# szpajder/dumphfdl

Measured on AMD Instinct MI355X. Metric: wideband I/Q Msamples/s (cf32 ingest -> decoded HFDL PDUs) at fixed channel count, higher is better.
Workload: dtype f32

## Files before the change

dumphfdl_amd/csrc/demod.h:

```cpp
#pragma once
#include <hip/hip_runtime.h>
#include <cstdint>
#include <cstddef>
#include <memory>
#include <vector>
#include "../../include/hfdl_gpu.h"
#include "hip_handles.h"
#include "kernels.h"

namespace hfdl {

struct ChanState;
struct ChanScalars;
struct FrameRec;

struct DemodImage;

struct Demod {
	int nch = 0, outs = 0, cap = 0;
	int batch = 1;
	uint32_t taken = 0, dropped = 0;
	uint64_t launches = 0, decodes = 0;
	bool separate_decode = false;
	int bounce_cap = 0;
	int pdu_cap = 0;
	bool taps_on = true;
	bool taps_enabled = true;
	size_t lds_bytes = 0;
	Stream st_collect;
	std::unique_ptr<DemodImage> img;
	DevBuf d_tables;
	DevArray<ChanState> d_states;
	DevArray<float2> d_data;
	DevArray<FrameRec> d_frames;
	DevArray<int> d_counts;
// ... 35 lines not shown
```

dumphfdl_amd/csrc/demod_core.h:

```cpp
#pragma once
#include <hip/hip_runtime.h>
#include "demod_logic.h"
#include "demod_lds.h"

namespace hfdl {

constexpr int DM_WAVES = 4, DM_THREADS = 64 * DM_WAVES;
constexpr int WAVE_AGC = 0, WAVE_TIMING = 1, WAVE_CARRIER = 2, WAVE_RESAMPLER = 3;

__device__ __forceinline__ float dpp_row_shr1(float old, float src)
{
	return __int_as_float(__builtin_amdgcn_update_dpp(__float_as_int(old), __float_as_int(src), 0x111, 0xf, 0xf, false));
}
__device__ __forceinline__ float dpp_row_shl1(float old, float src)
{
	return __int_as_float(__builtin_amdgcn_update_dpp(__float_as_int(old), __float_as_int(src), 0x101, 0xf, 0xf, false));
}
__device__ __forceinline__ float dpp_row_shl2(float old, float src)
{
	return __int_as_float(__builtin_amdgcn_update_dpp(__float_as_int(old), __float_as_int(src), 0x102, 0xf, 0xf, false));
}
__device__ __forceinline__ float dpp_row_ror1(float src)
{
	return __int_as_float(__builtin_amdgcn_update_dpp(0, __float_as_int(src), 0x121, 0xf, 0xf, false));
// ... 139 lines not shown
		io.mf[p] = v;
		if (p >= DM_RING - SS_HIST) io.mf[p - DM_RING] = v;
		if (TAPS) { io.tap_mf[k] = v; io.tap_level[k] = io.lvl[p]; }
	}
}


struct DemodInput {
	const cf *chan;
	size_t blk_stride;
	const int *ends;
	cf *ring;
	int n_in;
};

__device__ __forceinline__ cf input_sample(const DemodInput &in, int g)
{
	int b = 0, start = 0;
#pragma unroll
	for (int u = 0; u < DM_MAX_BLOCKS - 1; u++) {
		const int e = in.ends[u];
		if (g >= e) { b = u + 1; start = e; }
	}
	return in.chan[(size_t)b * in.blk_stride + (size_t)(g - start)];
}

template <bool TAPS>
__device__ __forceinline__ void resample_outputs(uint32_t rs_phase, const DemodConst &T, const BlockIo &io, const cf *ring, int k0, int k1, int lane)
{
	const int k = k0 + lane;
	if (k < k1) {
		const uint64_t t = (uint64_t)rs_phase + (uint64_t)k * T.rs_step;
		const int i = (int)(t >> 24);
		const float *h = T.rs_h + ((t & 0xFFFFFFu) >> 16) * D_RS_TAPS;
		float ar = 0, ai = 0;
		for (int j = 0; j < D_RS_TAPS; j++) {
			const cf x = ring[(i - j) & DM_IN_MASK];
// ... 501 lines not shown
	auto resampler_store = [&]() {
		cf nh;
		if (lane < D_RS_TAPS - 1) nh = in.ring[(n_in - 1 - lane) & DM_IN_MASK];
		__builtin_amdgcn_wave_barrier();
		if (lane < D_RS_TAPS - 1) a.rs_hist[lane] = nh;
		if (lane == 0) {
			S.rs_phase = (uint32_t)((uint64_t)rs_phase + (uint64_t)n_out * T.rs_step - total);
			if (TAPS) io.tap_counts[0] = n_out;
		}
	};

	if (tid < D_RS_TAPS - 1) in.ring[(-1 - tid) & DM_IN_MASK] = a.rs_hist[tid];
	if (wave == WAVE_TIMING && lane < D_MF - 1) io.agc[(-1 - lane) & DM_AGC_MASK] = a.mf_hist[lane];
	const int rs0 = n_out < DM_CHUNK ? n_out : DM_CHUNK;
	int in_loaded = need(rs0 + 2 * DM_CHUNK);
	for (int g = tid; g < in_loaded; g += DM_THREADS) in.ring[g & DM_IN_MASK] = input_sample(in, g);
	if (TAPS && tid == 0) io.tap_counts[1] = 0;
	__syncthreads();
	if (wave == WAVE_RESAMPLER) resample_outputs<TAPS>(rs_phase, T, io, in.ring, 0, rs0, lane);
	__syncthreads();
	if (n_out < 1) {
		if (wave == WAVE_RESAMPLER) resampler_store();
		return 0;
	}

	unsigned long long tP0 = __builtin_amdgcn_s_memtime();
	unsigned long long busy = 0;
	int nsym = 0;
	StepClock clk;
	StateProbe states;
	PipeProgress pp;
	pp.rs_ready = rs0;
	if (wave == WAVE_RESAMPLER) {
		for (int step = 0; pp.s3_done < n_out; step++) {
			PipeMail &mail = step_mail(sh.mbox, step);
			clk.begin<WAVE_RESAMPLER>();
			int to = pp.rs_ready;
			if (to < n_out) {
				to = resampler_advance(pp, n_out);
				const int hi = need(resampler_fetch_ahead(to, n_out));
				cf nx[2];
#pragma unroll
				for (int u = 0; u < 2; u++) {
					const int g = in_loaded + 64 * u + lane;
					nx[u] = g < hi ? input_sample(in, g) : cf{0.f, 0.f};
				}
				resample_outputs<TAPS>(rs_phase, T, io, in.ring, pp.rs_ready, to, lane);
#pragma unroll
				for (int u = 0; u < 2; u++) {
					const int g = in_loaded + 64 * u + lane;
					if (g < hi) in.ring[g & DM_IN_MASK] = nx[u];
				}
				for (int g = in_loaded + 128 + lane; g < hi; g += 64) in.ring[g & DM_IN_MASK] = input_sample(in, g);
				if (hi > in_loaded) in_loaded = hi;
			}
			if (lane == 0) mail.rs_ready = to;
			clk.end<WAVE_RESAMPLER>(busy, mail, lane);
			__syncthreads();
			pp.read(&mail);
		}
		resampler_store();
	} else if (wave == WAVE_AGC) {
		float agc_g = S.agc_g, agc_y2 = S.agc_y2;
		for (int step = 0; pp.s3_done < n_out; step++) {
			PipeMail &mail = step_mail(sh.mbox, step);
			clk.begin<WAVE_AGC>();
			int to = agc_advance(pp);
			if (to > pp.mf_ready) agc_mf_chunk<TAPS>(agc_g, agc_y2, T, io, pp.mf_ready, to, lane); else to = pp.mf_ready;
// ... 78 lines not shown
```

dumphfdl_amd/csrc/demod_host.cpp:

```cpp
#include <algorithm>
#include <cmath>
#include <cstdlib>
#include <cstring>
#include <vector>
#include "demod.h"
#include "demod_launch.h"
#include "demod_lds.h"
#include "demod_tables.h"

namespace hfdl {

struct DemodImage { DemodTables h; DevTables t; };

Demod::Demod() = default;
Demod::~Demod() = default;

static DevTables resolve_tables(const void *d_img, const DemodTables &h)
{
	const unsigned char *base = (const unsigned char *)d_img;
	auto at = [&](const void *field) { return base + ((const unsigned char *)field - (const unsigned char *)&h); };
	DevTables t;
	t.c.rs_h = (const float *)at(h.rs_h);
	t.c.rs_step = h.rs_step;
	t.c.mf = (const float *)at(h.mf);
// ... 1 lines not shown
	t.c.ss_dmf = (const float *)at(h.ss_dmf);
	t.c.lf_b0 = h.lf_b0; t.c.lf_a1 = h.lf_a1; t.c.ss_rate_adj = h.ss_rate_adj;
	t.c.eq_h0 = (const float *)at(h.eq_h0);
	t.c.a_hi = h.a_hi; t.c.a_lo = h.a_lo;
	t.c.m1_hi = (const uint64_t *)at(h.m1_hi);
	t.c.m1_lo = (const uint64_t *)at(h.m1_lo);
	t.scrambler = (const uint8_t *)at(h.scrambler);
	t.c.corr_tab = (const float *)at(h.corr_tab);
	t.c.psk_pts = (const float *)at(h.psk_pts);
	t.c.a1_lo = h.a1_lo; t.c.a1_hi = h.a1_hi; t.c.a2_lo = h.a2_lo; t.c.a2_hi = h.a2_hi; t.c.pos_min = h.pos_min;
	return t;
}

size_t Demod::workgroup_lds() { return demod_workgroup_lds(0); }

int Demod::fit_batch(int outs, float resamp_rate, int want)
{
	int batch = want < 1 ? 1 : (want > DM_MAX_BLOCKS ? DM_MAX_BLOCKS : want);
	for (;; batch--) {
		const int cap = (int)((double)outs * (double)batch * (double)resamp_rate + 8);
		if (batch > 1 && demod_workgroup_lds(cap) > 160 * 1024) continue;
		if (batch == 1 || (2 * cap <= 65535 && (double)cap / 5400.0 < 1.0)) break;
	}
	return batch;
}

int Demod::init(int nch_, int outs_, float resamp_rate, const int32_t *freqs, hipStream_t st, int batch_want)
{
	nch = nch_; outs = outs_;
	if (resamp_rate <= 0.5f || resamp_rate > 1.0f) return fail(HFDL_GPU_ERANGE, "resampling rate %g outside (0.5, 1]", (double)resamp_rate);
	batch = fit_batch(outs, resamp_rate, batch_want);
	cap = (int)((double)outs * (double)batch * (double)resamp_rate + 8);
	img = std::make_unique<DemodImage>();
	build_demod_tables(img->h, resamp_rate);
	CREATE_TRY(d_tables.alloc(sizeof(DemodTables)));
	CREATE_TRY(hipMemcpyAsync(d_tables.p, &img->h, sizeof(DemodTables), hipMemcpyHostToDevice, st));
	img->t = resolve_tables(d_tables.p, img->h);

	std::vector<ChanState> init((size_t)nch);
	for (auto &s : init) chan_state_init(s, img->h.eq_h0);
	CREATE_TRY(d_states.alloc((size_t)nch));
	CREATE_TRY(hipMemcpy(d_states, init.data(), sizeof(ChanState) * (size_t)nch, hipMemcpyHostToDevice));
	CREATE_TRY(d_data.alloc((size_t)nch * 2 * MAX_DATA_SYMBOLS));
	CREATE_TRY(hipMemsetAsync(d_data, 0, sizeof(float2) * (size_t)nch * 2 * MAX_DATA_SYMBOLS, st));
	CREATE_TRY(d_frames.alloc(2 * (size_t)nch));
	CREATE_TRY(d_counts.alloc(8));
	CREATE_TRY(hipMemsetAsync(d_counts, 0, sizeof(int) * 8, st));
	CREATE_TRY(h_snap.alloc(8));
	std::memset(h_snap.p, 0, sizeof(int) * 8);
	taken = 0; dropped = 0;
	pdu_cap = std::max(4096, 64 * nch);
	if (const char *e = getenv("HFDL_GPU_PDU_RING")) {
		const long v = strtol(e, nullptr, 10);
		if (v >= 1 && v <= (1 << 20)) pdu_cap = (int)v;
	}
	CREATE_TRY(d_pdus.alloc((size_t)pdu_cap));
	CREATE_TRY(st_collect.create());
	bounce_cap = pdu_cap < 512 ? pdu_cap : 512;
	CREATE_TRY(h_pdu_bounce.alloc((size_t)bounce_cap));
	CREATE_TRY(h_stats_bounce.alloc((size_t)nch));
// ... 7 lines not shown
		CREATE_TRY(d_tap_counts.alloc(2 * (size_t)nch));
		CREATE_TRY(hipMemsetAsync(d_tap_counts, 0, sizeof(int) * 2 * (size_t)nch, st));
	}
	lds_bytes = demod_workgroup_lds(cap);
	if (lds_bytes > 160 * 1024) return fail(HFDL_GPU_ERANGE, "a demodulator launch of %d samples needs %zu bytes of LDS", cap, lds_bytes);
	return prepare_demod_kernels(lds_bytes);
}

int Demod::enqueue_demod(const float2 *chan_out, const int *out_count, int nblk, hipStream_t st, hipEvent_t done, bool frames_free, hipEvent_t start)
{
	if (!img || nblk < 1 || nblk > batch || nblk > DM_MAX_BLOCKS)
		return fail(HFDL_GPU_EINVAL, "demodulator launch of %d blocks: 1 .. %d", nblk, batch);
	DemodBuffers B;
	const uint64_t i = launches++;
	if (separate_decode && !frames_free && ev_dec[i & 1]) HIP_TRY(hipStreamWaitEvent(st, ev_dec[i & 1], 0));
	B.states = d_states; B.data = (cf *)d_data.p; B.frames = d_frames + (size_t)(i & 1) * nch; B.counts = d_counts;
	B.frame_count = d_counts + 4 + (int)(i & 3); B.frame_cap = nch;
	const bool tw = taps_on && taps_enabled;
	B.tap_rs = tw ? (cf *)d_tap_rs.p : nullptr; B.tap_mf = (cf *)d_tap_mf.p; B.tap_sym = (cf *)d_tap_sym.p; B.tap_lvl = d_tap_lvl; B.tap_counts = d_tap_counts;
	B.cap = cap;
	launch_demod(tw, img->t, B, (const cf *)chan_out, out_count, outs, nblk, nch, lds_bytes, st, start, done);
	HIP_TRY(hipGetLastError());
	return 0;
}

int Demod::enqueue_decode(int buf, hipStream_t st, hipEvent_t start, hipEvent_t stop)
{
	if (!img) return fail(HFDL_GPU_EINVAL, "burst decoder launch before init");
	const uint64_t i = decodes++;
	if (i + 1 != launches) return fail(HFDL_GPU_EINVAL, "burst decoder launch %llu without its demodulator launch", (unsigned long long)i);
	launch_burst_decode(d_frames + (size_t)(i & 1) * nch, d_counts, d_counts + 4 + (int)(i & 3), d_counts + 4 + (int)((i + 2) & 3), nch,
			(const cf *)d_data.p, img->t.scrambler, d_freqs, d_pdus, pdu_cap, st, start, stop);
	HIP_TRY(hipMemcpyAsync(h_snap.p + 4 * (buf & 1), d_counts, sizeof(int) * 4, hipMemcpyDeviceToHost, st));
	if (separate_decode) {
		if (!ev_dec[i & 1]) HIP_TRY(ev_dec[i & 1].create(EV_NO_TIMING));
		HIP_TRY(hipEventRecord(ev_dec[i & 1], st));
	}
	HIP_TRY(hipGetLastError());
	return 0;
}

int Demod::prepare_retune(hipStream_t st_b)
{
	if (d_state_image.p) return 0;
	DevArray<ChanState> d;
	PinnedBuf<ChanState> h;
	Event ev;
// ... 122 lines not shown
```

dumphfdl_amd/csrc/demod_kernels.hip:

```cpp
#include <hip/hip_ext.h>
#include <utility>
#include "demod_core.h"
#ifdef HFDL_DM_STRICT
#include HFDL_DM_SERIAL_LOOP
#endif
#include "demod_tables.h"
#include "hip_handles.h"
#include "demod_launch.h"
#ifdef HFDL_LAB
#include "../../include/hfdl_gpu_lab.h"
#endif

namespace hfdl {

static_assert(sizeof(cf) == sizeof(float2), "cf must alias float2");

template <int NT, typename T>
__device__ __forceinline__ void stage_copy(T *__restrict__ dst, const T *__restrict__ src, int n, int tid)
{
	int i = tid;
	for (; i + 7 * NT < n; i += 8 * NT) {
		T v[8];
#pragma unroll
		for (int u = 0; u < 8; u++) v[u] = src[i + u * NT];
// ... 55 lines not shown
	if (tid < 8) { l_m1[tid] = T.c.m1_hi[tid]; l_m1[8 + tid] = T.c.m1_lo[tid]; }
	if (tid < 128) l_corr[tid] = T.c.corr_tab[tid];
	if (tid < (int)(2 * sizeof(PipeMail) / sizeof(int))) ((int *)(lds + L.mbox))[tid] = 0;
	__syncthreads();
	if (tid < DM_MAX_BLOCKS) {
		int sum = 0;
		for (int u = 0; u <= tid; u++) sum += l_blk[u];
		l_blk[DM_MAX_BLOCKS + tid] = sum;
	}
	__syncthreads();

	DemodConst K = T.c;
	K.rs_h = l_rs_h; K.ss_mf = nullptr; K.ss_dmf = nullptr; K.mf = l_mf; K.eq_h0 = l_eq; K.m1_hi = l_m1; K.m1_lo = l_m1 + 8; K.corr_tab = l_corr;
	BlockIo io;
	io.rs = (cf *)(lds + L.rs); io.agc = (cf *)(lds + L.agc); io.mf = (cf *)(lds + L.mfo); io.lvl = (float *)(lds + L.lvl); io.cap = B.cap;
	io.data = B.data + (size_t)c * 2 * MAX_DATA_SYMBOLS;
	io.frames = B.frames; io.frame_count = B.frame_count; io.frame_cap = B.frame_cap;
	io.channel = c;
	DemodInput in;
	in.chan = chan_out + (size_t)c * outs_stride; in.blk_stride = (size_t)nch * outs_stride;
	in.ends = l_blk + DM_MAX_BLOCKS; in.ring = (cf *)(lds + L.in); in.n_in = l_blk[2 * DM_MAX_BLOCKS - 1];
	if (TAPS) {
		io.tap_resampled = B.tap_rs + (size_t)c * B.cap; io.tap_mf = B.tap_mf + (size_t)c * B.cap;
		io.tap_symbols = B.tap_sym + (size_t)c * B.cap; io.tap_level = B.tap_lvl + (size_t)c * B.cap;
		io.tap_counts = B.tap_counts + 2 * c;
	} else {
		io.tap_resampled = nullptr; io.tap_mf = nullptr; io.tap_symbols = nullptr; io.tap_level = nullptr; io.tap_counts = nullptr;
	}
	DemodShared sh;
	sh.outq = (cf *)(lds + L.outq); sh.outq_cap = 2 * B.cap;
	sh.cum = (uint16_t *)(lds + L.cum);
// ... 167 lines not shown
	size_t table, vin, decw, consts, total;
	__host__ __device__ constexpr explicit BurstLds(bool viterbi)
		: table(0), vin(K5_TABLE_BYTES), decw(2 * (size_t)K5_TABLE_BYTES), consts(decw + (viterbi ? viterbi_lds_bytes(K5_MAX_BITS) : 0)), total(consts + DEC_CONST_BYTES) {}
};

struct BurstFrame {
	FrameRec fr;
	ModeParams mp;
	int nsym, ncoded, cols;
	const cf *sym;
	float mask_flip;
	uint8_t *l_scr;
	float *l_psk;
};

__device__ __forceinline__ BurstFrame burst_frame(const FrameRec *__restrict__ frames, int f, const cf *__restrict__ data_all, const uint8_t *__restrict__ scrambler,
		unsigned char *consts, int lane)
{
	BurstFrame b;
	b.l_scr = consts;
	b.l_psk = (float *)(consts + DEC_PSK_OFFSET);
	b.fr = frames[f];
	b.mp = mode_params(b.fr.mode);
	b.nsym = b.mp.segments * 30; b.ncoded = b.nsym * b.mp.arity; b.cols = b.ncoded / 40;
	b.sym = data_all + ((size_t)b.fr.channel * 2 + b.fr.slot) * MAX_DATA_SYMBOLS;
	b.mask_flip = b.fr.bitmask_lsb ? -1.0f : 1.0f;
	b.l_scr[lane] = lane < 120 ? scrambler[lane] : 0;
	if (lane + 64 < 120) b.l_scr[lane + 64] = scrambler[lane + 64];
	if (lane < 32) b.l_psk[lane] = ((const float *)(scrambler + DEC_PSK_OFFSET))[lane];
	__syncthreads();
	return b;
}

__device__ __forceinline__ int burst_soft_wave(const int mode, const int nsym, const int ncoded, const int cols, const cf *sym, const float mask_flip,
		const uint8_t *l_scr, const float *l_psk, uint8_t *table, uint8_t *vin)
{
	const int lane = threadIdx.x;
	const ModeParams mp = mode_params(mode);
	for (int base = 0; base < nsym; base += 256) {
		cf xs[4];
// ... 20 lines not shown
	__syncthreads();
	const int vin_len = mp.code_rate == 4 ? ncoded / 2 : ncoded;
	for (int j = lane; j < vin_len; j += 64) {
		if (mp.code_rate == 4) {
			const int p0 = 2 * j, p1 = 2 * j + 1;
			const uint8_t a = table[((9 * p0) % 40) * cols + p0 / 40], b = table[((9 * p1) % 40) * cols + p1 / 40];
			vin[j] = (uint8_t)((a & b) + ((a ^ b) >> 1));
		} else {
			vin[j] = table[((9 * j) % 40) * cols + j / 40];
		}
	}
	return vin_len;
}

__global__ __launch_bounds__(64) void burst_decode_kernel(const FrameRec *__restrict__ frames, int *counts, const int *nframes_ptr, int *stale_count, int frame_cap,
		const cf *__restrict__ data_all, const uint8_t *__restrict__ scrambler, const int32_t *__restrict__ freqs,
		hfdl_gpu_pdu *__restrict__ pdus, int pdu_cap)
{
	extern __shared__ __attribute__((aligned(16))) unsigned char lds[];
	__builtin_amdgcn_s_setprio(2);
	const int f = blockIdx.x, lane = threadIdx.x;
	int nframes = *nframes_ptr;
	if (f == 0 && lane == 0 && stale_count) *stale_count = 0;
	if (nframes > frame_cap) nframes = frame_cap;
	if (f >= nframes) return;
	constexpr BurstLds L(true);
	uint8_t *table = lds + L.table, *vin = lds + L.vin;
	uint64_t *decw = (uint64_t *)(lds + L.decw);
	const BurstFrame b = burst_frame(frames, f, data_all, scrambler, lds + L.consts, lane);
	const FrameRec &fr = b.fr;
	const ModeParams &mp = b.mp;
	const int vin_len = burst_soft_wave(fr.mode, b.nsym, b.ncoded, b.cols, b.sym, b.mask_flip, b.l_scr, b.l_psk, table, vin);
	int slot = -1;
	if (lane == 0) {
		unsigned *produced = (unsigned *)&counts[1];
		const unsigned taken = *(volatile unsigned *)&counts[3];
		unsigned t = *(volatile unsigned *)produced;
		for (;;) {
			if (t - taken >= (unsigned)pdu_cap) { atomicAdd(&counts[2], 1); break; }
			const unsigned seen = atomicCAS(produced, t, t + 1u);
			if (seen == t) { slot = (int)(t % (unsigned)pdu_cap); break; }
			t = seen;
		}
	}
// ... 29 lines not shown
		if (out->fcs_status == 0 && kind != 0) lc = lpdu_walk(l_oct, (uint32_t)noct, kind, hdr_len);
		out->lpdus_processed = lc.processed; out->lpdus_good = lc.good; out->lpdus_bad_fcs = lc.bad_fcs;
		out->lpdus_too_short = lc.too_short; out->lpdus_truncated = lc.truncated;
		out->lpdu_pad[0] = out->lpdu_pad[1] = out->lpdu_pad[2] = 0;
	}
}

#ifdef HFDL_LAB
__global__ __launch_bounds__(64) void burst_soft_kernel(const FrameRec *__restrict__ frames, const cf *__restrict__ data_all, const uint8_t *__restrict__ scrambler,
		uint8_t *__restrict__ vin_out, int32_t *__restrict__ vin_lens)
{
	extern __shared__ __attribute__((aligned(16))) unsigned char lds[];
	const int f = blockIdx.x, lane = threadIdx.x;
	constexpr BurstLds L(false);
	uint8_t *table = lds + L.table, *vin = lds + L.vin;
	const BurstFrame b = burst_frame(frames, f, data_all, scrambler, lds + L.consts, lane);
	const int vin_len = burst_soft_wave(b.fr.mode, b.nsym, b.ncoded, b.cols, b.sym, b.mask_flip, b.l_scr, b.l_psk, table, vin);
	__syncthreads();
	uint8_t *dst = vin_out + (size_t)f * HFDL_GPU_LAB_VIN_MAX;
	for (int j = lane; j < vin_len && j < HFDL_GPU_LAB_VIN_MAX; j += 64) dst[j] = vin[j];
	if (lane == 0) vin_lens[f] = vin_len;
}
#endif

__global__ __launch_bounds__(64) void viterbi_batch_kernel(const uint8_t *__restrict__ soft, int nbits, uint8_t *__restrict__ out)
{
	extern __shared__ __attribute__((aligned(16))) unsigned char lds[];
	const int f = blockIdx.x;
	viterbi27_wave(soft + (size_t)f * 2 * nbits, nbits, (uint64_t *)lds, out + (size_t)f * ((nbits + 7) / 8), false);
}

// ... 88 lines not shown
int prepare_demod_kernels(size_t demod_lds)
{
	int rc;
	if ((rc = set_big_lds((const void *)demod_kernel<true>, demod_lds))) return rc;
	if ((rc = set_big_lds((const void *)demod_kernel<false>, demod_lds))) return rc;
	return prepare_burst_decode();
}

void launch_demod(bool taps, const DevTables &T, const DemodBuffers &B, const cf *chan_out, const int *n_in, int outs_stride, int nblk, int nch,
		size_t lds, hipStream_t st, hipEvent_t start, hipEvent_t stop)
{
	if (taps) hipExtLaunchKernelGGL(demod_kernel<true>, dim3((unsigned)nch), dim3(DM_THREADS), (unsigned)lds, st, start, stop, 0, T, B, chan_out, n_in, outs_stride, nblk, nch);
	else hipExtLaunchKernelGGL(demod_kernel<false>, dim3((unsigned)nch), dim3(DM_THREADS), (unsigned)lds, st, start, stop, 0, T, B, chan_out, n_in, outs_stride, nblk, nch);
}

void launch_burst_decode(const FrameRec *frames, int *counts, const int *nframes, int *stale_count, int frame_cap, const cf *data,
		const uint8_t *scrambler, const int32_t *freqs, hfdl_gpu_pdu *pdus, int pdu_cap, hipStream_t st, hipEvent_t start, hipEvent_t stop)
{
	hipExtLaunchKernelGGL(burst_decode_kernel, dim3((unsigned)frame_cap), dim3(64), (unsigned)burst_decode_lds(), st, start, stop, 0, frames, counts,
			nframes, stale_count, frame_cap, data, scrambler, freqs, pdus, pdu_cap);
}

void launch_retune_demod(ChanState *states, const ChanState *image, int c, hipStream_t st, hipEvent_t done)
{
	hipExtLaunchKernelGGL(retune_demod_kernel, dim3(1), dim3(256), 0, st, nullptr, done, 0, states, image, c);
}

void launch_retune_freq(int32_t *freqs, int c, int32_t freq, hipStream_t st)
{
	hipLaunchKernelGGL(retune_freq_kernel, dim3(1), dim3(64), 0, st, freqs, c, freq);
}


int prepare_viterbi_batch(int nbits)
{
// ... 59 lines not shown
```

dumphfdl_amd/csrc/demod_launch.h:

```cpp
#pragma once
#include <hip/hip_runtime.h>
#include "../../include/hfdl_gpu.h"
#include "demod_logic.h"
#include "kernels.h"

namespace hfdl {

struct DevTables {
	DemodConst c;
	const uint8_t *scrambler;
};

struct DemodBuffers {
	ChanState *states;
	cf *data;
	FrameRec *frames;
	int *counts;
	int *frame_count;
	int frame_cap;
	cf *tap_rs, *tap_mf, *tap_sym;
	float *tap_lvl;
	int *tap_counts;
	int cap;
};

size_t demod_workgroup_lds(int cap);
size_t burst_decode_lds();
int prepare_demod_kernels(size_t demod_lds);
int prepare_burst_decode();
void launch_demod(bool taps, const DevTables &T, const DemodBuffers &B, const cf *chan_out, const int *n_in, int outs_stride, int nblk, int nch,
		size_t lds, hipStream_t st, hipEvent_t start, hipEvent_t stop);
void launch_burst_decode(const FrameRec *frames, int *counts, const int *nframes, int *stale_count, int frame_cap, const cf *data,
		const uint8_t *scrambler, const int32_t *freqs, hfdl_gpu_pdu *pdus, int pdu_cap, hipStream_t st, hipEvent_t start, hipEvent_t stop);
void launch_retune_demod(ChanState *states, const ChanState *image, int c, hipStream_t st, hipEvent_t done);
void launch_retune_freq(int32_t *freqs, int c, int32_t freq, hipStream_t st);
int read_device_constants(void *constants);

int prepare_viterbi_batch(int nbits);
void launch_viterbi_batch(const uint8_t *soft, int nbits, int nframes, uint8_t *out, hipStream_t st);
void launch_crc16(const uint8_t *data, uint32_t len, uint16_t crc_init, uint32_t *out, hipStream_t st);
void launch_pdu_triage(const uint8_t *octets, const int32_t *lens, int npdus, int stride, uint8_t *fcs_status, uint8_t *kind, uint16_t *hdr_len, hipStream_t st);
void launch_lpdu_walk(const uint8_t *octets, const int32_t *lens, int npdus, int stride, uint8_t *counts, hipStream_t st);
void launch_psk_slice(int arity, const cf *x, int n, const float *pts, uint32_t *sym, float *perr, hipStream_t st);
#ifdef HFDL_LAB
void launch_burst_soft(const FrameRec *frames, int nframes, const cf *data, const uint8_t *scrambler, uint8_t *vin, int32_t *vin_lens, hipStream_t st);
hipError_t demod_clock_probe_ring(ClockProbeRing &r);
#endif
// ... 3 lines not shown
```

dumphfdl_amd/csrc/demod_lds.h:

```cpp
#pragma once
#include <stddef.h>
#include <stdint.h>
#include "demod_logic.h"

namespace hfdl {

#ifndef HFDL_DM_CHUNK
#define HFDL_DM_CHUNK 32
#endif
constexpr int DM_CHUNK = HFDL_DM_CHUNK;
constexpr int OUTQ_RING = 512;
static_assert((OUTQ_RING & (OUTQ_RING - 1)) == 0 && OUTQ_RING >= 2 * DM_CHUNK * 4 + 64 + 64, "ring: a power of two that holds what can be live");

constexpr int SS_HIST = 34;
constexpr int DM_RING = 256, DM_MASK = DM_RING - 1;
constexpr int DM_MF_AHEAD = DM_RING - 2 * DM_CHUNK, DM_RS_AHEAD = DM_RING - DM_CHUNK;
static_assert(DM_MF_AHEAD + SS_HIST <= DM_RING && DM_MF_AHEAD >= 3 * DM_CHUNK, "matched-filter ring: history survives, and the pipeline in step (three chunks ahead) is never held back");
static_assert(DM_RS_AHEAD <= DM_RING && DM_RS_AHEAD >= DM_MF_AHEAD + DM_CHUNK, "resampler ring");
constexpr int DM_AGC_RING = 64, DM_AGC_MASK = DM_AGC_RING - 1;
static_assert(DM_AGC_RING >= DM_CHUNK + D_MF - 1 && DM_CHUNK <= 64, "AGC ring");
constexpr int DM_IN_RING = 256, DM_IN_MASK = DM_IN_RING - 1;
static_assert(DM_IN_RING >= 3 * (2 * DM_CHUNK + 1) + D_RS_TAPS, "input ring");
constexpr int DM_MAX_BLOCKS = 7;
constexpr size_t DM_LDS_BUDGET = 40 * 1024;

struct PipeMail {
	int mf_ready;
	int ss_ready;
	int s3_done;
	int s3_reset;
	int rs_ready;
	int busy[3];
};

struct PipeProgress {
	int rs_ready = 0, mf_ready = 0, ss_ready = 0, s3_done = 0;
	bool restart = false;
	__host__ __device__ inline void read(const PipeMail *m)
// ... 87 lines not shown
```

dumphfdl_amd/csrc/demod_logic.h:

```cpp
#pragma once
#include <stdint.h>
#include <math.h>

#define HFDL_FN __device__ inline
#define HFDL_HD __host__ __device__ inline
#ifndef HFDL_ATAN2F
#define HFDL_ATAN2F atan2f
#endif

namespace hfdl {

struct cf { float x, y; };

constexpr int D_RS_NPFB = 256, D_RS_TAPS = 14, D_SS_NPFB = 16, D_SS_TAPS = 18, D_EQ = 15, D_MF = 19;
constexpr int MAX_DATA_SYMBOLS = 168 * 30;

constexpr int PREKEY_LEN = 448, A_LEN = 127, M1_LEN = 127, M2_LEN = 15, T_LEN = 15, DATA_FRAME_LEN = 30, PREAMBLE_T_SEQS = 9;
constexpr int SINGLE_SLOT_FRAME_LEN = PREKEY_LEN + (2 * A_LEN + M1_LEN + M2_LEN + PREAMBLE_T_SEQS * T_LEN) + 72 * (DATA_FRAME_LEN + T_LEN);
constexpr float CORR_THRESHOLD_A1 = 0.36f, CORR_THRESHOLD_A2 = 0.3f, CORR_THRESHOLD_M1 = 0.3f;
constexpr int MAX_SEARCH_RETRIES = 3, NO_FRAME_TIMEOUT_FRAMES = 13;
constexpr int HFDL_SYMBOL_RATE = 1800, HFDL_SPS = 3;
constexpr float COSTAS_ALPHA = 0.1f, COSTAS_BETA = 0.047f * COSTAS_ALPHA * COSTAS_ALPHA;
constexpr float COSTAS_ERR_LIMIT = 1.0f, COSTAS_RUNAWAY_DPHI = 0.25f;
constexpr float AGC_BANDWIDTH = 0.01f, EQ_STEP = 0.1f;
// ... 62 lines not shown
	const float *ss_mf, *ss_dmf;
	float lf_b0, lf_a1, ss_rate_adj;
	const float *eq_h0;
	uint64_t a_hi, a_lo;
	const uint64_t *m1_hi, *m1_lo;
	const float *corr_tab;
	const float *psk_pts;
	int32_t a1_lo, a1_hi, a2_lo, a2_hi, pos_min;
};

struct BlockIo {
	cf *rs, *agc, *mf;
	float *lvl;
	int cap;
	cf *data;
	FrameRec *frames;
	int *frame_count;
	int frame_cap;
	cf *tap_resampled, *tap_mf, *tap_symbols;
	float *tap_level;
	int *tap_counts;
	int channel;
};

#ifndef HFDL_DM_SS_RATE0
#define HFDL_DM_SS_RATE0 1.5f
#endif

HFDL_HD void chan_state_init(ChanState &st, const float *eq_h0)
{
// ... 346 lines not shown
			s.fr_state = FR_DATA_1;
			s.cur_arity = c.data_arity;
			s.use_data = 1;
		} else {
			if ((threadIdx.x & 63u) == 0) {
				const int slot = atomicAdd(io.frame_count, 1);
				if (slot < io.frame_cap) {
					FrameRec fr;
					fr.channel = io.channel; fr.slot = s.data_slot; fr.mode = c.M1; fr.bitmask_lsb = (int32_t)(s.bitmask & 1u);
					fr.freq_err_hz = c.freq_err_hz; fr.signal_level = s.signal_level; fr.noise_floor = s.noise_floor;
					fr.train_bad = c.train_bad; fr.train_total = c.train_total; fr.pad = 0;
					fr.sample_index = c.pdu_sample_index;
					io.frames[slot] = fr;
				}
			}
			s.data_slot ^= 1;
			c.cnt_frames++;
			framer_reset(s, c, a, T.eq_h0);
			s.symbol_cnt = 0;
		}
		break; }
	case FR_DATA_1:
		s.symbols_wanted = DATA_FRAME_LEN / 2;
		s.fr_state = FR_DATA_2;
		break;
	case FR_DATA_2:
		c.data_segment_cnt--;
		s.cur_arity = 1;
		s.use_data = 0;
		s.fr_state = FR_EQ_TRAIN;
		c.eq_train_seq_cnt = 1;
// ... 37 lines not shown
```

dumphfdl_amd/csrc/frontend_create.cpp:

```cpp
#include <atomic>
#include <cmath>
#include <complex>
#include <cstring>
#include <thread>
#include "frontend.h"

using namespace hfdl;

extern "C" int hfdl_gpu_device_count(void)
{
	int n = 0;
	if (hipGetDeviceCount(&n) != hipSuccess) return 0;
	return n;
}

int hfdl::select_device(int device)
{
	int n = 0;
	if (hipGetDeviceCount(&n) != hipSuccess || n <= 0)
		return fail(HFDL_GPU_ENODEV, "no HIP device visible: the HFDL front end has no CPU fallback");
	if (device < 0 || device >= n) return fail(HFDL_GPU_EINVAL, "device %d out of range (%d visible)", device, n);
	HIP_TRY(hipSetDevice(device));
	hipDeviceProp_t prop;
	HIP_TRY(hipGetDeviceProperties(&prop, device));
// ... 205 lines not shown
	g.nch = nch;
	g.tap_layout = (pl.m % 16) == 0 && (pl.pre % 8) == 0 ? TAPL_OCTET : TAPL_PLAIN;
	g.nch_pad = plan_receiver_slots(nch_per_rx, nrx, tap_layout_group(g.tap_layout), fe->rx_span);
	for (const RxSpan &r : fe->rx_span) fe->rx_host.push_back(make_int4(r.slot0, r.slots, r.chan0, r.nch));
	g.nrx = nrx;
	g.spec_rx_stride = pl.n;
	g.rx_host = fe->rx_host.data();
	g.tap_chan_stride = pl.m; g.tap_row_stride = (int64_t)g.nch_pad * pl.m;
	g.fold_tile = lab.fold_tile;
	fe->tap_layout.kind = g.tap_layout;
	fe->tap_layout.row_log = ilog2(pl.m); fe->tap_layout.row_stride = g.tap_row_stride;
	fe->prune_tol = g.tap_layout == TAPL_OCTET && nrx == 1 ? env_double("HFDL_GPU_FOLD_PRUNE", 1e-12, 1e-3, 0.0) : 0.0;
	fe->fold_bound = lab.fold_bound < 0 ? nch >= 128 : lab.fold_bound != 0;
	const float resamp_rate = (float)(1800 * 3) / ((float)fe->sample_rate / (float)fe->decimation);
	BatchOverrides ov;
	ov.demod_batch = (int)env_long("HFDL_GPU_DEMOD_BATCH", 1, 8, 0);
	ov.fold_batch = (int)env_long("HFDL_GPU_FOLD_BATCH", 1, hfdl_gpu_frontend::MAX_HALF, 0);
	ov.pruned = fe->prune_tol > 0;
	ov.fold_slices = lab.fold_slices;
	ov.no_ramp = !lab.fold_ramp;
	const BatchPlan bp = plan_batches(nch, nrx, pl.n, pl.input_size, fe->sample_rate, pl.pre, fe->fold_bound,
			[&](int want) { return Demod::fit_batch(g.outs, resamp_rate, want); }, ov);
	g.slices = bp.slices;
	g.rows_per_slice = pl.pre / g.slices;
	if (pl.m > 8192 || pl.m < 16) return fail(HFDL_GPU_ERANGE, "inverse FFT size %d unsupported", pl.m);

	if (int rc = create_streams(fe, lab)) return rc;
	for (int i = 0; i < 2; i++) {
		CREATE_TRY(fe->spec[i].own.create(EV_NO_TIMING));
		CREATE_TRY(fe->chan[i].own.create(EV_NO_TIMING));
		CREATE_TRY(fe->ev_demod[i].create(EV_NO_TIMING));
// ... 89 lines not shown
```

dumphfdl_amd/csrc/planner.h:

```cpp
#pragma once
#include <algorithm>
#include <cmath>
#include <cstdint>
#include <vector>
#include <complex>

namespace hfdl {

struct Plan {
	int32_t pre, post, taps_min_length, taps_length, overlap, n, m, input_size, post_input_size, scrap, v;
	int32_t startbin, offsetbin;
	float pre_shift, post_shift, sindelta, cosdelta, rate;
};

inline int32_t pow2_above(int32_t x)
{
	int32_t p = 1;
	for (int i = 0; i < 31; i++, p <<= 1) if (x < p) return p;
	return -1;
}

inline int32_t fft_decimation_rate(int32_t fs, int32_t target)
{
	return pow2_above((int32_t)std::floor((float)fs / (float)target)) / 2;
// ... 134 lines not shown
constexpr int PLAN_MAX_HALF = 32;
constexpr int PLAN_MAX_STAGE = 18;

template <typename Fit>
inline BatchPlan plan_batches(int nch, int nrx, int n, int input_size, int sample_rate, int pre, bool fold_bound, Fit demod_fit, const BatchOverrides &ov)
{
	BatchPlan b{};
	b.slices = pick_slices(nch, pre);
	if (ov.fold_slices > 0 && (ov.fold_slices & (ov.fold_slices - 1)) == 0 && pre % ov.fold_slices == 0 && pre / ov.fold_slices >= 16) b.slices = ov.fold_slices;
	if (ov.pruned) b.slices = 1;

	b.fold_nb = ov.fold_batch ? ov.fold_batch : (fold_bound ? 32 : 8);

	int want = (int)std::floor(1.0 / ((double)input_size / (double)sample_rate));
	want = std::max(1, std::min(8, want));
	if (fold_bound) want = std::min(want, 3);
	if (ov.demod_batch) want = ov.demod_batch;
	want = demod_fit(want);
	if (nrx > 1) {
		const int64_t cap = std::max<int64_t>(1, ((int64_t)32 << 23) / ((int64_t)nrx * (int64_t)n));
		if (cap < std::max(b.fold_nb, want)) {
			b.fold_nb = (int)std::min<int64_t>(b.fold_nb, cap);
			want = std::min(want, b.fold_nb);
		}
	}
	if (!ov.demod_batch && want < b.fold_nb) {
		const int launches = (b.fold_nb + want - 1) / want;
		want = (b.fold_nb + launches - 1) / launches;
	}
	b.batch_want = want;
	const int batch = demod_fit(want);
	b.half_blocks = std::min(PLAN_MAX_HALF, ((std::max(b.fold_nb, batch) + b.fold_nb - 1) / b.fold_nb) * b.fold_nb);
	b.half_first = (fold_bound && b.half_blocks > 16 && !ov.no_ramp) ? 16 : b.half_blocks;
	b.n_stage = std::min(b.half_blocks + 2, PLAN_MAX_STAGE);
	return b;
}


enum FftSide { FFT_SERIAL = 0, FFT_BESIDE = 1 };
enum FftRule { FFT_RULE_INPUT, FFT_RULE_SERIAL, FFT_RULE_OWN };
inline int fft_side(FftRule rule, bool on_device) { return rule == FFT_RULE_INPUT ? (on_device ? FFT_BESIDE : FFT_SERIAL) : rule == FFT_RULE_OWN ? FFT_BESIDE : FFT_SERIAL; }

struct FftPushPlan { int side; bool wait_switch, wait_set_free, wait_first_fold, flush_before, hold_after, wait_retune; };
struct HalfClosePlan { bool wait_input, hold_back; };
struct FftOrder {
	int prev_side = -1;
	bool half_beside = false;
	int halves = 0;
	bool retuned = false;
	FftPushPlan push(int side, int fill, int target, bool held_back)
// ... 93 lines not shown
```

dumphfdl_amd/csrc/stages.cpp:

```cpp
#include <cmath>
#include <cstring>
#include <vector>
#include "frontend.h"
#include "demod_launch.h"
#include "demod_tables.h"

using namespace hfdl;

static thread_local double g_stage_ms = 0.0;
extern "C" double hfdl_gpu_last_stage_ms(void) { return g_stage_ms; }

int hfdl::finish_stage()
{
	HIP_TRY(hipDeviceSynchronize());
	HIP_TRY(hipGetLastError());
	return 0;
}

int StageFrames::upload(const float *symbols, const int32_t *modes, const int32_t *bitmask_lsb, int32_t nframes)
{
	DemodTables h;
	build_demod_tables(h, 0.6912f);
	std::vector<FrameRec> fr((size_t)nframes);
	std::vector<cf> sym((size_t)nframes * 2 * MAX_DATA_SYMBOLS);
// ... 58 lines not shown
{
	if (!symbols || !modes || !bitmask_lsb || !octets || !lens || nframes <= 0) return fail(HFDL_GPU_EINVAL, "bad arguments");
	for (int i = 0; i < nframes; i++) if (modes[i] < 0 || modes[i] > 7) return fail(HFDL_GPU_EINVAL, "mode out of range");
	int rc = select_device(device);
	if (rc) return rc;
	g_stage_ms = 0.0;
	StageFrames in;
	if ((rc = in.upload(symbols, modes, bitmask_lsb, nframes))) return rc;
	const int counts[8] = { 0, 0, 0, 0, nframes, 0, 0, 0 };
	DevBuf d_counts, d_freqs, d_pdus;
	HIP_TRY(d_counts.upload(counts, sizeof(counts)));
	HIP_TRY(d_freqs.zeroed(sizeof(int32_t) * (size_t)nframes));
	HIP_TRY(d_pdus.alloc(sizeof(hfdl_gpu_pdu) * (size_t)nframes));
	if ((rc = prepare_burst_decode())) return rc;
	StageTimer tm;
	launch_burst_decode(in.frames.as<const FrameRec>(), d_counts.as<int>(), d_counts.as<int>() + 4, nullptr, nframes, in.data.as<const cf>(),
			in.scrambler.as<const uint8_t>(), d_freqs.as<const int32_t>(), d_pdus.as<hfdl_gpu_pdu>(), nframes, nullptr, nullptr, nullptr);
	g_stage_ms = tm.stop();
	if ((rc = finish_stage())) return rc;
	std::vector<hfdl_gpu_pdu> pdus((size_t)nframes);
	HIP_TRY(d_pdus.fetch(pdus.data(), sizeof(hfdl_gpu_pdu) * pdus.size()));
	for (int i = 0; i < nframes; i++) lens[i] = 0;
	for (auto &p : pdus) {
		if (p.channel < 0 || p.channel >= nframes) continue;
		lens[p.channel] = p.len;
		std::memcpy(octets + (size_t)p.channel * HFDL_GPU_PDU_MAX_OCTETS, p.octets, (size_t)p.len);
	}
	return 0;
}

extern "C" int hfdl_gpu_nco_decimate(int device, const float *in, int32_t input_size, float rate, int32_t decimation,
// ... 104 lines not shown
```

Measured before the change: 21900.

## Allow larger demod batches with multi-slot frame buffers and block cursor input lookup

Raises the maximum number of input blocks per demodulator launch from 7 to 32 and drops the fold-bound cap of three blocks, so each demod launch can span a whole fold half. Per-channel frame and data slots are now sized from the launch duration, so several frames can complete within one launch without overwriting each other. The input sample lookup walks a wave-uniform block cursor instead of a fixed unrolled scan over all block ends. The aim is fewer demod and decode launches per unit of input. The cost is more LDS and memory for the larger capacity, longer per-launch latency, and a burst decode grid that grows with frames per channel.

```diff
diff --git a/dumphfdl_amd/csrc/demod.h b/dumphfdl_amd/csrc/demod.h
--- a/dumphfdl_amd/csrc/demod.h
+++ b/dumphfdl_amd/csrc/demod.h
@@ -19,6 +19,7 @@
 struct Demod {
 	int nch = 0, outs = 0, cap = 0;
 	int batch = 1;
+	int frames_per_chan = 1, data_slots = 2;
 	uint32_t taken = 0, dropped = 0;
 	uint64_t launches = 0, decodes = 0;
 	bool separate_decode = false;
diff --git a/dumphfdl_amd/csrc/demod_core.h b/dumphfdl_amd/csrc/demod_core.h
--- a/dumphfdl_amd/csrc/demod_core.h
+++ b/dumphfdl_amd/csrc/demod_core.h
@@ -177,13 +177,22 @@
 	int n_in;
 };
 
-__device__ __forceinline__ cf input_sample(const DemodInput &in, int g)
-{
-	int b = 0, start = 0;
-#pragma unroll
-	for (int u = 0; u < DM_MAX_BLOCKS - 1; u++) {
-		const int e = in.ends[u];
-		if (g >= e) { b = u + 1; start = e; }
+struct BlockCursor {
+	int b = 0, start = 0, end = 0;
+	__device__ __forceinline__ void begin(const DemodInput &in) { b = 0; start = 0; end = __builtin_amdgcn_readfirstlane(in.ends[0]); }
+	__device__ __forceinline__ void advance(const DemodInput &in, int g)
+	{
+		g = __builtin_amdgcn_readfirstlane(g);
+		while (g >= end && b < DM_MAX_BLOCKS - 1) { start = end; b++; end = __builtin_amdgcn_readfirstlane(in.ends[b]); }
+	}
+};
+
+__device__ __forceinline__ cf input_sample(const DemodInput &in, const BlockCursor &at, int g)
+{
+	int b = at.b, start = at.start;
+	if (__builtin_expect(g >= at.end, 0)) {
+		int e = at.end;
+		do { start = e; b++; e = in.ends[b]; } while (g >= e && b < DM_MAX_BLOCKS - 1);
 	}
 	return in.chan[(size_t)b * in.blk_stride + (size_t)(g - start)];
 }
@@ -715,7 +724,9 @@
 	if (wave == WAVE_TIMING && lane < D_MF - 1) io.agc[(-1 - lane) & DM_AGC_MASK] = a.mf_hist[lane];
 	const int rs0 = n_out < DM_CHUNK ? n_out : DM_CHUNK;
 	int in_loaded = need(rs0 + 2 * DM_CHUNK);
-	for (int g = tid; g < in_loaded; g += DM_THREADS) in.ring[g & DM_IN_MASK] = input_sample(in, g);
+	BlockCursor at;
+	at.begin(in);
+	for (int g = tid; g < in_loaded; g += DM_THREADS) in.ring[g & DM_IN_MASK] = input_sample(in, at, g);
 	if (TAPS && tid == 0) io.tap_counts[1] = 0;
 	__syncthreads();
 	if (wave == WAVE_RESAMPLER) resample_outputs<TAPS>(rs_phase, T, io, in.ring, 0, rs0, lane);
@@ -740,11 +751,12 @@
 			if (to < n_out) {
 				to = resampler_advance(pp, n_out);
 				const int hi = need(resampler_fetch_ahead(to, n_out));
+				at.advance(in, in_loaded);
 				cf nx[2];
 #pragma unroll
 				for (int u = 0; u < 2; u++) {
 					const int g = in_loaded + 64 * u + lane;
-					nx[u] = g < hi ? input_sample(in, g) : cf{0.f, 0.f};
+					nx[u] = g < hi ? input_sample(in, at, g) : cf{0.f, 0.f};
 				}
 				resample_outputs<TAPS>(rs_phase, T, io, in.ring, pp.rs_ready, to, lane);
 #pragma unroll
@@ -752,7 +764,7 @@
 					const int g = in_loaded + 64 * u + lane;
 					if (g < hi) in.ring[g & DM_IN_MASK] = nx[u];
 				}
-				for (int g = in_loaded + 128 + lane; g < hi; g += 64) in.ring[g & DM_IN_MASK] = input_sample(in, g);
+				for (int g = in_loaded + 128 + lane; g < hi; g += 64) in.ring[g & DM_IN_MASK] = input_sample(in, at, g);
 				if (hi > in_loaded) in_loaded = hi;
 			}
 			if (lane == 0) mail.rs_ready = to;
diff --git a/dumphfdl_amd/csrc/demod_host.cpp b/dumphfdl_amd/csrc/demod_host.cpp
--- a/dumphfdl_amd/csrc/demod_host.cpp
+++ b/dumphfdl_amd/csrc/demod_host.cpp
@@ -7,6 +7,7 @@
 #include "demod_launch.h"
 #include "demod_lds.h"
 #include "demod_tables.h"
+#include "planner.h"
 
 namespace hfdl {
 
@@ -39,14 +40,12 @@
 
 size_t Demod::workgroup_lds() { return demod_workgroup_lds(0); }
 
+static_assert(DM_MAX_BLOCKS == PLAN_MAX_HALF, "a half that closes full is one demodulator launch");
+
 int Demod::fit_batch(int outs, float resamp_rate, int want)
 {
-	int batch = want < 1 ? 1 : (want > DM_MAX_BLOCKS ? DM_MAX_BLOCKS : want);
-	for (;; batch--) {
-		const int cap = (int)((double)outs * (double)batch * (double)resamp_rate + 8);
-		if (batch > 1 && demod_workgroup_lds(cap) > 160 * 1024) continue;
-		if (batch == 1 || (2 * cap <= 65535 && (double)cap / 5400.0 < 1.0)) break;
-	}
+	int batch = fit_output_counts(outs, resamp_rate, want);
+	while (batch > 1 && demod_workgroup_lds(demod_launch_samples(outs, batch, resamp_rate)) > 160 * 1024) batch--;
 	return batch;
 }
 
@@ -55,7 +54,9 @@
 	nch = nch_; outs = outs_;
 	if (resamp_rate <= 0.5f || resamp_rate > 1.0f) return fail(HFDL_GPU_ERANGE, "resampling rate %g outside (0.5, 1]", (double)resamp_rate);
 	batch = fit_batch(outs, resamp_rate, batch_want);
-	cap = (int)((double)outs * (double)batch * (double)resamp_rate + 8);
+	cap = demod_launch_samples(outs, batch, resamp_rate);
+	const FrameSlots fs = plan_frame_slots((double)cap / 5400.0);
+	frames_per_chan = fs.per_channel; data_slots = fs.data_slots;
 	img = std::make_unique<DemodImage>();
 	build_demod_tables(img->h, resamp_rate);
 	CREATE_TRY(d_tables.alloc(sizeof(DemodTables)));
@@ -66,9 +67,9 @@
 	for (auto &s : init) chan_state_init(s, img->h.eq_h0);
 	CREATE_TRY(d_states.alloc((size_t)nch));
 	CREATE_TRY(hipMemcpy(d_states, init.data(), sizeof(ChanState) * (size_t)nch, hipMemcpyHostToDevice));
-	CREATE_TRY(d_data.alloc((size_t)nch * 2 * MAX_DATA_SYMBOLS));
-	CREATE_TRY(hipMemsetAsync(d_data, 0, sizeof(float2) * (size_t)nch * 2 * MAX_DATA_SYMBOLS, st));
-	CREATE_TRY(d_frames.alloc(2 * (size_t)nch));
+	CREATE_TRY(d_data.alloc((size_t)nch * data_slots * MAX_DATA_SYMBOLS));
+	CREATE_TRY(hipMemsetAsync(d_data, 0, sizeof(float2) * (size_t)nch * data_slots * MAX_DATA_SYMBOLS, st));
+	CREATE_TRY(d_frames.alloc(2 * (size_t)nch * frames_per_chan));
 	CREATE_TRY(d_counts.alloc(8));
 	CREATE_TRY(hipMemsetAsync(d_counts, 0, sizeof(int) * 8, st));
 	CREATE_TRY(h_snap.alloc(8));
@@ -106,8 +107,8 @@
 	DemodBuffers B;
 	const uint64_t i = launches++;
 	if (separate_decode && !frames_free && ev_dec[i & 1]) HIP_TRY(hipStreamWaitEvent(st, ev_dec[i & 1], 0));
-	B.states = d_states; B.data = (cf *)d_data.p; B.frames = d_frames + (size_t)(i & 1) * nch; B.counts = d_counts;
-	B.frame_count = d_counts + 4 + (int)(i & 3); B.frame_cap = nch;
+	B.states = d_states; B.data = (cf *)d_data.p; B.data_slots = data_slots; B.frames = d_frames + (size_t)(i & 1) * nch * frames_per_chan; B.counts = d_counts;
+	B.frame_count = d_counts + 4 + (int)(i & 3); B.frame_cap = nch * frames_per_chan;
 	const bool tw = taps_on && taps_enabled;
 	B.tap_rs = tw ? (cf *)d_tap_rs.p : nullptr; B.tap_mf = (cf *)d_tap_mf.p; B.tap_sym = (cf *)d_tap_sym.p; B.tap_lvl = d_tap_lvl; B.tap_counts = d_tap_counts;
 	B.cap = cap;
@@ -121,8 +122,8 @@
 	if (!img) return fail(HFDL_GPU_EINVAL, "burst decoder launch before init");
 	const uint64_t i = decodes++;
 	if (i + 1 != launches) return fail(HFDL_GPU_EINVAL, "burst decoder launch %llu without its demodulator launch", (unsigned long long)i);
-	launch_burst_decode(d_frames + (size_t)(i & 1) * nch, d_counts, d_counts + 4 + (int)(i & 3), d_counts + 4 + (int)((i + 2) & 3), nch,
-			(const cf *)d_data.p, img->t.scrambler, d_freqs, d_pdus, pdu_cap, st, start, stop);
+	launch_burst_decode(d_frames + (size_t)(i & 1) * nch * frames_per_chan, d_counts, d_counts + 4 + (int)(i & 3), d_counts + 4 + (int)((i + 2) & 3), nch * frames_per_chan,
+			(const cf *)d_data.p, data_slots, img->t.scrambler, d_freqs, d_pdus, pdu_cap, st, start, stop);
 	HIP_TRY(hipMemcpyAsync(h_snap.p + 4 * (buf & 1), d_counts, sizeof(int) * 4, hipMemcpyDeviceToHost, st));
 	if (separate_decode) {
 		if (!ev_dec[i & 1]) HIP_TRY(ev_dec[i & 1].create(EV_NO_TIMING));
diff --git a/dumphfdl_amd/csrc/demod_kernels.hip b/dumphfdl_amd/csrc/demod_kernels.hip
--- a/dumphfdl_amd/csrc/demod_kernels.hip
+++ b/dumphfdl_amd/csrc/demod_kernels.hip
@@ -93,7 +93,7 @@
 	K.rs_h = l_rs_h; K.ss_mf = nullptr; K.ss_dmf = nullptr; K.mf = l_mf; K.eq_h0 = l_eq; K.m1_hi = l_m1; K.m1_lo = l_m1 + 8; K.corr_tab = l_corr;
 	BlockIo io;
 	io.rs = (cf *)(lds + L.rs); io.agc = (cf *)(lds + L.agc); io.mf = (cf *)(lds + L.mfo); io.lvl = (float *)(lds + L.lvl); io.cap = B.cap;
-	io.data = B.data + (size_t)c * 2 * MAX_DATA_SYMBOLS;
+	io.data = B.data + (size_t)c * B.data_slots * MAX_DATA_SYMBOLS; io.data_slots = B.data_slots;
 	io.frames = B.frames; io.frame_count = B.frame_count; io.frame_cap = B.frame_cap;
 	io.channel = c;
 	DemodInput in;
@@ -291,8 +291,8 @@
 	float *l_psk;
 };
 
-__device__ __forceinline__ BurstFrame burst_frame(const FrameRec *__restrict__ frames, int f, const cf *__restrict__ data_all, const uint8_t *__restrict__ scrambler,
-		unsigned char *consts, int lane)
+__device__ __forceinline__ BurstFrame burst_frame(const FrameRec *__restrict__ frames, int f, const cf *__restrict__ data_all, int data_slots,
+		const uint8_t *__restrict__ scrambler, unsigned char *consts, int lane)
 {
 	BurstFrame b;
 	b.l_scr = consts;
@@ -300,7 +300,7 @@
 	b.fr = frames[f];
 	b.mp = mode_params(b.fr.mode);
 	b.nsym = b.mp.segments * 30; b.ncoded = b.nsym * b.mp.arity; b.cols = b.ncoded / 40;
-	b.sym = data_all + ((size_t)b.fr.channel * 2 + b.fr.slot) * MAX_DATA_SYMBOLS;
+	b.sym = data_all + ((size_t)b.fr.channel * data_slots + b.fr.slot) * MAX_DATA_SYMBOLS;
 	b.mask_flip = b.fr.bitmask_lsb ? -1.0f : 1.0f;
 	b.l_scr[lane] = lane < 120 ? scrambler[lane] : 0;
 	if (lane + 64 < 120) b.l_scr[lane + 64] = scrambler[lane + 64];
@@ -351,7 +351,7 @@
 }
 
 __global__ __launch_bounds__(64) void burst_decode_kernel(const FrameRec *__restrict__ frames, int *counts, const int *nframes_ptr, int *stale_count, int frame_cap,
-		const cf *__restrict__ data_all, const uint8_t *__restrict__ scrambler, const int32_t *__restrict__ freqs,
+		const cf *__restrict__ data_all, int data_slots, const uint8_t *__restrict__ scrambler, const int32_t *__restrict__ freqs,
 		hfdl_gpu_pdu *__restrict__ pdus, int pdu_cap)
 {
 	extern __shared__ __attribute__((aligned(16))) unsigned char lds[];
@@ -364,7 +364,7 @@
 	constexpr BurstLds L(true);
 	uint8_t *table = lds + L.table, *vin = lds + L.vin;
 	uint64_t *decw = (uint64_t *)(lds + L.decw);
-	const BurstFrame b = burst_frame(frames, f, data_all, scrambler, lds + L.consts, lane);
+	const BurstFrame b = burst_frame(frames, f, data_all, data_slots, scrambler, lds + L.consts, lane);
 	const FrameRec &fr = b.fr;
 	const ModeParams &mp = b.mp;
 	const int vin_len = burst_soft_wave(fr.mode, b.nsym, b.ncoded, b.cols, b.sym, b.mask_flip, b.l_scr, b.l_psk, table, vin);
@@ -424,7 +424,7 @@
 	const int f = blockIdx.x, lane = threadIdx.x;
 	constexpr BurstLds L(false);
 	uint8_t *table = lds + L.table, *vin = lds + L.vin;
-	const BurstFrame b = burst_frame(frames, f, data_all, scrambler, lds + L.consts, lane);
+	const BurstFrame b = burst_frame(frames, f, data_all, 2, scrambler, lds + L.consts, lane);
 	const int vin_len = burst_soft_wave(b.fr.mode, b.nsym, b.ncoded, b.cols, b.sym, b.mask_flip, b.l_scr, b.l_psk, table, vin);
 	__syncthreads();
 	uint8_t *dst = vin_out + (size_t)f * HFDL_GPU_LAB_VIN_MAX;
@@ -543,11 +543,11 @@
 	else hipExtLaunchKernelGGL(demod_kernel<false>, dim3((unsigned)nch), dim3(DM_THREADS), (unsigned)lds, st, start, stop, 0, T, B, chan_out, n_in, outs_stride, nblk, nch);
 }
 
-void launch_burst_decode(const FrameRec *frames, int *counts, const int *nframes, int *stale_count, int frame_cap, const cf *data,
+void launch_burst_decode(const FrameRec *frames, int *counts, const int *nframes, int *stale_count, int frame_cap, const cf *data, int data_slots,
 		const uint8_t *scrambler, const int32_t *freqs, hfdl_gpu_pdu *pdus, int pdu_cap, hipStream_t st, hipEvent_t start, hipEvent_t stop)
 {
 	hipExtLaunchKernelGGL(burst_decode_kernel, dim3((unsigned)frame_cap), dim3(64), (unsigned)burst_decode_lds(), st, start, stop, 0, frames, counts,
-			nframes, stale_count, frame_cap, data, scrambler, freqs, pdus, pdu_cap);
+			nframes, stale_count, frame_cap, data, data_slots, scrambler, freqs, pdus, pdu_cap);
 }
 
 void launch_retune_demod(ChanState *states, const ChanState *image, int c, hipStream_t st, hipEvent_t done)
diff --git a/dumphfdl_amd/csrc/demod_launch.h b/dumphfdl_amd/csrc/demod_launch.h
--- a/dumphfdl_amd/csrc/demod_launch.h
+++ b/dumphfdl_amd/csrc/demod_launch.h
@@ -14,6 +14,7 @@
 struct DemodBuffers {
 	ChanState *states;
 	cf *data;
+	int data_slots;
 	FrameRec *frames;
 	int *counts;
 	int *frame_count;
@@ -30,7 +31,7 @@
 int prepare_burst_decode();
 void launch_demod(bool taps, const DevTables &T, const DemodBuffers &B, const cf *chan_out, const int *n_in, int outs_stride, int nblk, int nch,
 		size_t lds, hipStream_t st, hipEvent_t start, hipEvent_t stop);
-void launch_burst_decode(const FrameRec *frames, int *counts, const int *nframes, int *stale_count, int frame_cap, const cf *data,
+void launch_burst_decode(const FrameRec *frames, int *counts, const int *nframes, int *stale_count, int frame_cap, const cf *data, int data_slots,
 		const uint8_t *scrambler, const int32_t *freqs, hfdl_gpu_pdu *pdus, int pdu_cap, hipStream_t st, hipEvent_t start, hipEvent_t stop);
 void launch_retune_demod(ChanState *states, const ChanState *image, int c, hipStream_t st, hipEvent_t done);
 void launch_retune_freq(int32_t *freqs, int c, int32_t freq, hipStream_t st);
diff --git a/dumphfdl_amd/csrc/demod_lds.h b/dumphfdl_amd/csrc/demod_lds.h
--- a/dumphfdl_amd/csrc/demod_lds.h
+++ b/dumphfdl_amd/csrc/demod_lds.h
@@ -21,7 +21,7 @@
 static_assert(DM_AGC_RING >= DM_CHUNK + D_MF - 1 && DM_CHUNK <= 64, "AGC ring");
 constexpr int DM_IN_RING = 256, DM_IN_MASK = DM_IN_RING - 1;
 static_assert(DM_IN_RING >= 3 * (2 * DM_CHUNK + 1) + D_RS_TAPS, "input ring");
-constexpr int DM_MAX_BLOCKS = 7;
+constexpr int DM_MAX_BLOCKS = 32;
 constexpr size_t DM_LDS_BUDGET = 40 * 1024;
 
 struct PipeMail {
diff --git a/dumphfdl_amd/csrc/demod_logic.h b/dumphfdl_amd/csrc/demod_logic.h
--- a/dumphfdl_amd/csrc/demod_logic.h
+++ b/dumphfdl_amd/csrc/demod_logic.h
@@ -100,6 +100,7 @@
 	float *lvl;
 	int cap;
 	cf *data;
+	int data_slots = 2;
 	FrameRec *frames;
 	int *frame_count;
 	int frame_cap;
@@ -476,7 +477,7 @@
 					io.frames[slot] = fr;
 				}
 			}
-			s.data_slot ^= 1;
+			s.data_slot = s.data_slot + 1 < io.data_slots ? s.data_slot + 1 : 0;
 			c.cnt_frames++;
 			framer_reset(s, c, a, T.eq_h0);
 			s.symbol_cnt = 0;
diff --git a/dumphfdl_amd/csrc/frontend_create.cpp b/dumphfdl_amd/csrc/frontend_create.cpp
--- a/dumphfdl_amd/csrc/frontend_create.cpp
+++ b/dumphfdl_amd/csrc/frontend_create.cpp
@@ -243,7 +243,7 @@
 	fe->fold_bound = lab.fold_bound < 0 ? nch >= 128 : lab.fold_bound != 0;
 	const float resamp_rate = (float)(1800 * 3) / ((float)fe->sample_rate / (float)fe->decimation);
 	BatchOverrides ov;
-	ov.demod_batch = (int)env_long("HFDL_GPU_DEMOD_BATCH", 1, 8, 0);
+	ov.demod_batch = (int)env_long("HFDL_GPU_DEMOD_BATCH", 1, hfdl_gpu_frontend::MAX_HALF, 0);
 	ov.fold_batch = (int)env_long("HFDL_GPU_FOLD_BATCH", 1, hfdl_gpu_frontend::MAX_HALF, 0);
 	ov.pruned = fe->prune_tol > 0;
 	ov.fold_slices = lab.fold_slices;
diff --git a/dumphfdl_amd/csrc/planner.h b/dumphfdl_amd/csrc/planner.h
--- a/dumphfdl_amd/csrc/planner.h
+++ b/dumphfdl_amd/csrc/planner.h
@@ -172,7 +172,7 @@
 
 	int want = (int)std::floor(1.0 / ((double)input_size / (double)sample_rate));
 	want = std::max(1, std::min(8, want));
-	if (fold_bound) want = std::min(want, 3);
+	want = std::max(want, b.fold_nb);
 	if (ov.demod_batch) want = ov.demod_batch;
 	want = demod_fit(want);
 	if (nrx > 1) {
@@ -192,6 +192,23 @@
 	b.half_first = (fold_bound && b.half_blocks > 16 && !ov.no_ramp) ? 16 : b.half_blocks;
 	b.n_stage = std::min(b.half_blocks + 2, PLAN_MAX_STAGE);
 	return b;
+}
+
+
+inline int demod_launch_samples(int outs, int batch, float rate) { return (int)((double)outs * (double)batch * (double)rate + 8); }
+inline int fit_output_counts(int outs, float rate, int want)
+{
+	int batch = std::max(1, std::min(PLAN_MAX_HALF, want));
+	while (batch > 1 && 2 * demod_launch_samples(outs, batch, rate) > 65535) batch--;
+	return batch;
+}
+
+
+constexpr double PLAN_MIN_FRAME_S = 3771.0 / 1800.0;
+struct FrameSlots { int per_channel, data_slots; };
+inline FrameSlots plan_frame_slots(double t_launch, double t_frame = PLAN_MIN_FRAME_S)
+{
+	return FrameSlots{ (int)std::floor(t_launch / t_frame) + 1, (int)std::floor(2.0 * t_launch / t_frame) + 2 };
 }
 
 
diff --git a/dumphfdl_amd/csrc/stages.cpp b/dumphfdl_amd/csrc/stages.cpp
--- a/dumphfdl_amd/csrc/stages.cpp
+++ b/dumphfdl_amd/csrc/stages.cpp
@@ -96,7 +96,7 @@
 	HIP_TRY(d_pdus.alloc(sizeof(hfdl_gpu_pdu) * (size_t)nframes));
 	if ((rc = prepare_burst_decode())) return rc;
 	StageTimer tm;
-	launch_burst_decode(in.frames.as<const FrameRec>(), d_counts.as<int>(), d_counts.as<int>() + 4, nullptr, nframes, in.data.as<const cf>(),
+	launch_burst_decode(in.frames.as<const FrameRec>(), d_counts.as<int>(), d_counts.as<int>() + 4, nullptr, nframes, in.data.as<const cf>(), 2,
 			in.scrambler.as<const uint8_t>(), d_freqs.as<const int32_t>(), d_pdus.as<hfdl_gpu_pdu>(), nframes, nullptr, nullptr, nullptr);
 	g_stage_ms = tm.stop();
 	if ((rc = finish_stage())) return rc;
```

After: 22420, median of 6. 2.4% higher.
